# FelixWaiblinger/gym-pybullet-adrp

Measured on AMD Instinct MI355X. Metric: env-steps/sec (N parallel drones) at 1/2/4/8 MI355X; % HBM roofline, higher is better.
Workload: dtype f64; 1 GPU; HoverAviary Physics.PYB 240/30 Hz (8 sub-steps), 4096 envs x 1 drone per GPU, RPM actions, auto-reset; envs_per_gpu=4096, global_envs=4096, drones_per_env=1, parallelism=env-sharded dp1

## Files before the change

### gym_pybullet_adrp_amd/csrc/hover_kernel.h

```cpp
#pragma once

#include "adrp_device.h"
#include "dslpid_core.h"

namespace adrp {

enum HoverField {
    HF_POS = 0, HF_QUAT = 3, HF_VEL = 7, HF_OMEGA = 10, HF_LAST_RPM = 13, HF_ANGV = 17,
    HF_LINK_QUAT = 20, HF_NBASE = 24,
    HF_PID = 24, HF_NPID = 9
};
enum HoverInt { HI_STEP = 0, HI_EPISODE = 1, HI_RING_HEAD = 2, HI_N = 3 };

template <typename Real>
struct HoverConst {
    int S, trunc_steps, link_lag, physics;
    Real dt, mass, inv_mass, gravity;
    Real ixx, iyy, izz, inv_ixx, inv_iyy, inv_izz;
    Real kf, km, hover_rpm;
    Real px[4], py[4], pz[4];
    Real gnd_kf, prop_r4, gnd_clip;
    Real drag[3];
    Real dyn_arm;
    Real coll_hh, coll_r, coll_zoff;
// ... 20 lines not shown
    c.dyn_arm = Real(0.028072139213105935);
    c.coll_hh = Real(0.0125); c.coll_r = Real(0.06); c.coll_zoff = Real(0);
    c.ang_max = Real(188.49555921538757);
    c.target[0] = Real(0); c.target[1] = Real(0); c.target[2] = Real(1);
    c.pid_grav = Real(0.338492); c.pid_inv4kf = Real(791139240.5063292);
    c.ctrl_dt = Real(0.03333333333333333); c.ctrl_hz = Real(30);
    c.speed_limit = 0.25f;
    return c;
}

template <typename Real>
struct HoverReset {
    Real init_xyz[3], init_rpy[3], n_xyz[3], n_rpy[3], n_vel[3], n_om[3];
};

constexpr int kStepBlock = 64;
constexpr int kResetFields = 16;
#ifndef ADRP_PERSIST_SPLIT
#define ADRP_PERSIST_SPLIT 1
#endif
#ifndef ADRP_HOVER_ANGLE_HELPERS
#define ADRP_HOVER_ANGLE_HELPERS 1
#endif
template <typename Real>
constexpr bool angle_helpers() { return ADRP_HOVER_ANGLE_HELPERS != 0 && sizeof(Real) == 8; }
template <typename Real>
constexpr int help_waves() { return angle_helpers<Real>() ? 3 : 1; }

template <typename Real>
struct HoverArgs {
    const HoverConst<Real>* c;
    const HoverReset<Real>* r;
    Real* f;
    float* ring;
    int32_t* ist;
    const float* act;
    float* obs;
    float* rew;
    uint8_t* term;
    uint8_t* trunc;
    float* tobs;
    const uint8_t* mask;
    int32_t* contact_count;
    uint64_t seed;
    int64_t env_offset;
    int E, B, D, autoreset;
// ... 35 lines not shown
}
template <typename Real>
__device__ __forceinline__ V3<Real> row2_fm(Q4<Real> q) {
    const Real x2 = q.x + q.x, y2 = q.y + q.y, z2 = q.z + q.z;
    const Real xx = q.x * x2;
    const Real wx = q.w * x2, wy = q.w * y2;
    return {fmx(q.x, z2, -wy), fmx(q.y, z2, wx), Real(1) - fmx(q.y, y2, xx)};
}

template <typename Real>
struct Chain {
    V3<Real> wb;
    Real wn;
    V3<Real> zs;
    V3<Real> zc;
    V3<Real> m3;
    V3<Real> dti;
    M3<Real> R, Rs;
};

__device__ __forceinline__ float clamp100_(float x) { return __builtin_amdgcn_fmed3f(x, -100.0f, 100.0f); }
__device__ __forceinline__ double clamp100_(double x) { return clamp100_sel(x); }

template <typename Real>
__device__ __forceinline__ void clamp100_body(Q4<Real> q, V3<Real>& wb, Real& wn, V3<Real>& v, const ChainK<Real>& K) {
    const Real c = K.c100;
    const bool fast = wn > c;
    bool big = fast;
    if constexpr (sizeof(Real) == 8) {
        const bool bx = fabs_(v.x) > c, by = fabs_(v.y) > c, bz = fabs_(v.z) > c;
        big = fast | bx | by | bz;
    } else {
        v = v3(clamp100_(v.x), clamp100_(v.y), clamp100_(v.z));
    }
    if (__builtin_expect(__any(big), 0)) {
        if constexpr (sizeof(Real) == 8) v = v3(clamp100_(v.x), clamp100_(v.y), clamp100_(v.z));
        const M3<Real> R = rot_fm(q);
        const V3<Real> w = mul(R, wb);
        const V3<Real> wc = mulT(R, v3(clamp100_(w.x), clamp100_(w.y), clamp100_(w.z)));
        const Real wnc = hsqrt_nn_(dot(wc, wc), K);
        wb = v3(fast ? wc.x : wb.x, fast ? wc.y : wb.y, fast ? wc.z : wb.z);
        wn = fast ? wnc : wn;
    }
}

template <typename Real>
__device__ __forceinline__ bool flat_props(const HoverConst<Real>& a) {
    bool flat = true;
#pragma unroll
    for (int i = 0; i < 4; ++i) flat = flat && __builtin_constant_p(a.pz[i]) && a.pz[i] == Real(0);
    return flat;
}

template <typename Real, int PH, bool EXT = false>
__device__ __forceinline__ bool pyb_substep(const HoverConst<Real>& a, Body<Real>& b, Chain<Real>& st,
                                            const Real rpm[4], Real sum_f, V3<Real> P, Real tau_z,
                                            const ChainK<Real>& K, V3<Real> Fext = V3<Real>{}, Real* vxy = nullptr) {
    constexpr bool GND = (PH == ADRP_PHYS_PYB_GND || PH == ADRP_PHYS_PYB_GND_DRAG_DW);
    constexpr bool DRAG = (PH == ADRP_PHYS_PYB_DRAG || PH == ADRP_PHYS_PYB_GND_DRAG_DW);
    constexpr bool FULL = DRAG && !GND;
    const V3<Real> zs = st.zs;
    V3<Real> Fw = v3(sum_f * zs.x, sum_f * zs.y, sum_f * zs.z - a.mass * a.gravity);
    const V3<Real> m3 = st.m3;
    V3<Real> nb = flat_props(a)
                      ? v3(fmx(tau_z, m3.x, P.y * m3.z), fmx(tau_z, m3.y, -(P.x * m3.z)),
                           fmx(tau_z, m3.z, fmx(P.x, m3.y, -(P.y * m3.x))))
                      : v3(fmx(tau_z, m3.x, fmx(P.y, m3.z, -(P.z * m3.y))), fmx(tau_z, m3.y, fmx(P.z, m3.x, -(P.x * m3.z))),
                           fmx(tau_z, m3.z, fmx(P.x, m3.y, -(P.y * m3.x))));
    if constexpr (GND) {
        const Real sqx = b.q.x * b.q.x, sqy = b.q.y * b.q.y, sqz = b.q.z * b.q.z, squ = b.q.w * b.q.w;
        const Real sarg = Real(-2) * (b.q.x * b.q.z - b.q.w * b.q.y);
        const Real den = squ - sqx - sqy + sqz, num = Real(2) * (b.q.y * b.q.z + b.q.w * b.q.x);
        const bool gate = fabs_(sarg) < Real(0.99999) && (den > Real(0) || (den == Real(0) && num == Real(0)));
        if (gate) {
            Real sg = 0;
            V3<Real> G = v3(Real(0), Real(0), Real(0));
            const V3<Real> r2 = row2_fm(b.q);
#pragma unroll
            for (int i = 0; i < 4; ++i) {
                Real h = b.pos.z + r2.x * a.px[i] + r2.y * a.py[i] + r2.z * a.pz[i];
                h = h < a.gnd_clip ? a.gnd_clip : h;
                const Real k = a.prop_r4 * rcp_(h);
                const Real g = a.gnd_kf * rpm[i] * rpm[i] * k * k;
                sg += g;
                G = G + v3(g * a.px[i], g * a.py[i], g * a.pz[i]);
            }
            Fw = Fw + sg * st.zc;
            nb = nb + v3(G.y, -G.x, Real(0));
        }
    }
    if constexpr (DRAG) {
        Real s = 0;
#pragma unroll
        for (int i = 0; i < 4; ++i) s += b.prev_rpm[i];
        s = s * Real(0.10471975511965977);
        const V3<Real> dw = v3(-a.drag[0] * s * b.vel.x, -a.drag[1] * s * b.vel.y, -a.drag[2] * s * b.vel.z);
        if constexpr (GND) Fw = Fw + dw;
        else Fw = Fw + mul(st.Rs, mulT(st.R, dw));
    }
    if constexpr (EXT) Fw = Fw + Fext;
    V3<Real> wb = st.wb;
    const V3<Real> Iw = v3(a.ixx * wb.x, a.iyy * wb.y, a.izz * wb.z);
    const Real kw = K.k004 + K.k004 * st.wn;
    const V3<Real> rhs = v3(fmx(wb.z, Iw.y, fmx(-wb.y, Iw.z, fmx(-kw, Iw.x, nb.x))),
                            fmx(wb.x, Iw.z, fmx(-wb.z, Iw.x, fmx(-kw, Iw.y, nb.y))),
                            fmx(wb.y, Iw.x, fmx(-wb.x, Iw.y, fmx(-kw, Iw.z, nb.z))));
    const Real kv = K.k004 + K.k004 * hsqrt_nn_(dot(b.vel, b.vel), K);
    const V3<Real> acc = v3(fmx(-kv, b.vel.x, a.inv_mass * Fw.x), fmx(-kv, b.vel.y, a.inv_mass * Fw.y),
                            fmx(-kv, b.vel.z, a.inv_mass * Fw.z));
    wb = v3(fmx(st.dti.x, rhs.x, wb.x), fmx(st.dti.y, rhs.y, wb.y), fmx(st.dti.z, rhs.z, wb.z));
    b.vel = v3(b.vel.x + a.dt * acc.x, b.vel.y + a.dt * acc.y, b.vel.z + a.dt * acc.z);
    Real ang = hsqrt_nn_(dot(wb, wb), K);
    clamp100_body(b.q, wb, ang, b.vel, K);
    st.wb = wb;
    st.wn = ang;
    if (vxy) {
        vxy[0] = b.vel.x; vxy[1] = b.vel.y;
        b.pos.z = fmx(a.dt, b.vel.z, b.pos.z);
    } else {
        b.pos = v3(fmx(a.dt, b.vel.x, b.pos.x), fmx(a.dt, b.vel.y, b.pos.y), fmx(a.dt, b.vel.z, b.pos.z));
    }
    if (ang > a.ang_max) ang = a.ang_max;
    Real sinc, ch;
    expmap_sinc_cos(Real(0.5) * ang * a.dt, &sinc, &ch, K);
    const Real sc = (Real(0.5) * a.dt) * sinc;
    const V3<Real> ax = sc * wb;
    const Q4<Real> q0 = b.q;
    const Q4<Real> q1 = {ch * q0.x + ax.x * q0.w + ax.z * q0.y - ax.y * q0.z,
                         ch * q0.y + ax.y * q0.w + ax.x * q0.z - ax.z * q0.x,
                         ch * q0.z + ax.z * q0.w + ax.y * q0.x - ax.x * q0.y,
                         ch * q0.w - ax.x * q0.x - ax.y * q0.y - ax.z * q0.z};
    const Real inv = quat_inv_norm(q1.x * q1.x + q1.y * q1.y + q1.z * q1.z + q1.w * q1.w, K);
    if (a.link_lag) {
        b.ql = q0;
        st.zs = st.zc;
        const Real s2 = (inv + inv) * inv;
        st.m3 = v3(s2 * (ax.x * ax.z - ch * ax.y), s2 * (ax.y * ax.z + ch * ax.x),
                   Real(1) - s2 * (ax.x * ax.x + ax.y * ax.y));
        if constexpr (FULL) st.Rs = st.R;
    }
    b.q = {q1.x * inv, q1.y * inv, q1.z * inv, q1.w * inv};
    if constexpr (FULL) {
        st.R = rot_fm(b.q);
        st.zc = col2(st.R);
    } else {
        st.zc = col2_fm(b.q);
    }
    if (!a.link_lag) {
        st.zs = st.zc;
        st.m3 = v3(Real(0), Real(0), Real(1));
        if constexpr (FULL) st.Rs = st.R;
    }
    if (__builtin_expect(__any(b.pos.z + a.coll_zoff <= a.coll_hh + a.coll_r + Real(1e-6)), 0)) {
        const Real low = b.pos.z + a.coll_zoff - a.coll_hh * fabs_(st.zc.z) -
                         a.coll_r * hsqrt_nn_(st.zc.x * st.zc.x + st.zc.y * st.zc.y);
        if (low < Real(0)) {
            b.pos.z -= low;
            if (b.vel.z < Real(0)) b.vel.z = Real(0);
            return true;
        }
    }
    return false;
}

template <typename Real>
__device__ __forceinline__ void dyn_substep(const HoverConst<Real>& a, Body<Real>& b, const Real rpm[4]) {
    const M3<Real> R = rot(b.q);
    Real f[4], zt[4], sum = 0;
#pragma unroll
    for (int i = 0; i < 4; ++i) {
        f[i] = rpm[i] * rpm[i] * a.kf;
        zt[i] = rpm[i] * rpm[i] * a.km;
        sum += f[i];
    }
    const V3<Real> zb = col2(R);
    const V3<Real> force_w = v3(sum * zb.x, sum * zb.y, sum * zb.z - a.gravity * a.mass);
    const Real tz = -zt[0] + zt[1] - zt[2] + zt[3];
    const Real tx = (f[0] + f[1] - f[2] - f[3]) * a.dyn_arm;
    const Real ty = (-f[0] + f[1] + f[2] - f[3]) * a.dyn_arm;
    const V3<Real> rr = b.w;
    const V3<Real> tq = v3(tx, ty, tz) - cross(rr, v3(a.ixx * rr.x, a.iyy * rr.y, a.izz * rr.z));
    const V3<Real> rdd = v3(tq.x * a.inv_ixx, tq.y * a.inv_iyy, tq.z * a.inv_izz);
    b.vel = b.vel + a.dt * (a.inv_mass * force_w);
// ... 276 lines not shown
#pragma unroll
    for (int i = 0; i < n; ++i) {
        o[first + i] = off;
        if (i + 1 < n) off = field_lane(off + stride);
    }
}
template <typename Real>
struct BodyOffs {
    uint32_t o[HF_NBASE];
};
template <typename Real>
__device__ __forceinline__ BodyOffs<Real> body_offsets(int E, int e, bool lag, bool drag, bool dyn) {
    BodyOffs<Real> r;
    const uint32_t stride = uint32_t(E) * uint32_t(sizeof(Real)), off0 = uint32_t(e) * uint32_t(sizeof(Real));
    field_run(off0, stride, HF_POS, HF_LAST_RPM - HF_POS, r.o);
    if (drag) field_run(off0, stride, HF_LAST_RPM, 4, r.o);
    if (dyn) field_run(off0, stride, HF_ANGV, 3, r.o);
    if (lag) field_run(off0, stride, HF_LINK_QUAT, 4, r.o);
    return r;
}

template <typename Real>
__device__ __forceinline__ void load_body_at(const Real* f, const BodyOffs<Real>& k, Body<Real>& b, bool lag,
                                             bool drag, bool dyn) {
    b.pos = v3(field_at(f, k.o[HF_POS + 0]), field_at(f, k.o[HF_POS + 1]), field_at(f, k.o[HF_POS + 2]));
    b.q = {field_at(f, k.o[HF_QUAT + 0]), field_at(f, k.o[HF_QUAT + 1]), field_at(f, k.o[HF_QUAT + 2]),
           field_at(f, k.o[HF_QUAT + 3])};
    b.vel = v3(field_at(f, k.o[HF_VEL + 0]), field_at(f, k.o[HF_VEL + 1]), field_at(f, k.o[HF_VEL + 2]));
    b.w = v3(field_at(f, k.o[HF_OMEGA + 0]), field_at(f, k.o[HF_OMEGA + 1]), field_at(f, k.o[HF_OMEGA + 2]));
    if (lag) b.ql = {field_at(f, k.o[HF_LINK_QUAT + 0]), field_at(f, k.o[HF_LINK_QUAT + 1]),
                     field_at(f, k.o[HF_LINK_QUAT + 2]), field_at(f, k.o[HF_LINK_QUAT + 3])};
    else b.ql = b.q;
#pragma unroll
    for (int i = 0; i < 4; ++i) b.prev_rpm[i] = drag ? field_at(f, k.o[HF_LAST_RPM + i]) : Real(0);
    if (dyn) b.angv = v3(field_at(f, k.o[HF_ANGV + 0]), field_at(f, k.o[HF_ANGV + 1]), field_at(f, k.o[HF_ANGV + 2]));
    else b.angv = v3(Real(0), Real(0), Real(0));
}
template <typename Real>
__device__ __forceinline__ void store_body_at(Real* f, const BodyOffs<Real>& k, const Body<Real>& b, bool lag,
                                              bool drag, bool dyn) {
    field_last(f, k.o[HF_POS + 0]) = b.pos.x; field_last(f, k.o[HF_POS + 1]) = b.pos.y; field_last(f, k.o[HF_POS + 2]) = b.pos.z;
    field_last(f, k.o[HF_QUAT + 0]) = b.q.x; field_last(f, k.o[HF_QUAT + 1]) = b.q.y;
    field_last(f, k.o[HF_QUAT + 2]) = b.q.z; field_last(f, k.o[HF_QUAT + 3]) = b.q.w;
    field_last(f, k.o[HF_VEL + 0]) = b.vel.x; field_last(f, k.o[HF_VEL + 1]) = b.vel.y; field_last(f, k.o[HF_VEL + 2]) = b.vel.z;
    field_last(f, k.o[HF_OMEGA + 0]) = b.w.x; field_last(f, k.o[HF_OMEGA + 1]) = b.w.y; field_last(f, k.o[HF_OMEGA + 2]) = b.w.z;
    if (lag) {
        field_last(f, k.o[HF_LINK_QUAT + 0]) = b.ql.x; field_last(f, k.o[HF_LINK_QUAT + 1]) = b.ql.y;
        field_last(f, k.o[HF_LINK_QUAT + 2]) = b.ql.z; field_last(f, k.o[HF_LINK_QUAT + 3]) = b.ql.w;
    }
    if (drag) {
#pragma unroll
// ... 37 lines not shown
        store_body_at(f, body_offsets<Real>(E, e, lag, drag, dyn), b, lag, drag, dyn);
        field_form_end();
        return;
    }
    f[(HF_POS + 0) * E + e] = b.pos.x; f[(HF_POS + 1) * E + e] = b.pos.y; f[(HF_POS + 2) * E + e] = b.pos.z;
    f[(HF_QUAT + 0) * E + e] = b.q.x; f[(HF_QUAT + 1) * E + e] = b.q.y;
    f[(HF_QUAT + 2) * E + e] = b.q.z; f[(HF_QUAT + 3) * E + e] = b.q.w;
    f[(HF_VEL + 0) * E + e] = b.vel.x; f[(HF_VEL + 1) * E + e] = b.vel.y; f[(HF_VEL + 2) * E + e] = b.vel.z;
    f[(HF_OMEGA + 0) * E + e] = b.w.x; f[(HF_OMEGA + 1) * E + e] = b.w.y; f[(HF_OMEGA + 2) * E + e] = b.w.z;
    if (lag) {
        f[(HF_LINK_QUAT + 0) * E + e] = b.ql.x; f[(HF_LINK_QUAT + 1) * E + e] = b.ql.y;
        f[(HF_LINK_QUAT + 2) * E + e] = b.ql.z; f[(HF_LINK_QUAT + 3) * E + e] = b.ql.w;
    }
    if (drag) {
#pragma unroll
        for (int i = 0; i < 4; ++i) f[(HF_LAST_RPM + i) * E + e] = b.prev_rpm[i];
    }
    if (dyn) {
        f[(HF_ANGV + 0) * E + e] = b.angv.x; f[(HF_ANGV + 1) * E + e] = b.angv.y; f[(HF_ANGV + 2) * E + e] = b.angv.z;
    }
}

struct NoExtForce {};
template <typename Real, int PH, int SC, bool DRAG, typename Ext>
__device__ __forceinline__ bool pyb_chain(const HoverConst<Real>& C, Body<Real>& b, const Real rpm_in[4], bool lag,
                                          Ext ext, V3<Real>* wb_out = nullptr, Real* vxy = nullptr) {
    constexpr bool EXT = !__is_same(Ext, NoExtForce);
    const Real rpm[4] = {rpm_in[0], rpm_in[1], rpm_in[2], rpm_in[3]};
    Real sum_f = 0, t2 = 0;
    V3<Real> P = v3(Real(0), Real(0), Real(0));
#pragma unroll
    for (int i = 0; i < 4; ++i) {
        const Real r2 = rpm[i] * rpm[i];
        const Real f = r2 * C.kf;
        sum_f += f;
        const bool pz0 = __builtin_constant_p(C.pz[i]) && C.pz[i] == Real(0);
        const Real fx = f * C.px[i], fy = f * C.py[i], fz = f * C.pz[i];
        P = v3(P.x + fx, P.y + fy, pz0 ? P.z : P.z + fz);
        t2 += (i & 1) ? -r2 : r2;
    }
    const Real tau_z = t2 * C.km;
    ChainK<Real> K = chain_consts<Real>();
    HoverConst<Real> Cp = C;
    if constexpr (sizeof(Real) == 8) {
        pin_all(K);
        pin(Cp.dt); pin(Cp.mass); pin(Cp.gravity); pin(Cp.inv_mass); pin(Cp.ang_max);
        pin(Cp.ixx); pin(Cp.iyy); pin(Cp.izz); pin(Cp.inv_ixx); pin(Cp.inv_iyy); pin(Cp.inv_izz);
        pin(Cp.coll_hh); pin(Cp.coll_r); pin(Cp.coll_zoff);
    }
    Chain<Real> st{};
    {
        const M3<Real> R = rot_fm(b.q);
        const M3<Real> Rs = lag ? rot_fm(b.ql) : R;
        st.wb = mulT(R, b.w);
        st.zc = col2(R);
        st.zs = col2(Rs);
        st.m3 = lag ? mulT(R, st.zs) : v3(Real(0), Real(0), Real(1));
        if constexpr (DRAG) {
            st.R = R;
            st.Rs = Rs;
        }
    }
    st.wn = hsqrt_nn_(dot(b.w, b.w), K);
    st.dti = v3(Cp.dt * Cp.inv_ixx, Cp.dt * Cp.inv_iyy, Cp.dt * Cp.inv_izz);
    bool touched = false;
    auto substep = [&](int s) {
        if constexpr (EXT) touched |= pyb_substep<Real, PH, true>(Cp, b, st, rpm, sum_f, P, tau_z, K, ext(b, st));
        else touched |= pyb_substep<Real, PH>(Cp, b, st, rpm, sum_f, P, tau_z, K, V3<Real>{}, vxy ? vxy + 2 * s : nullptr);
#pragma unroll
        for (int i = 0; i < 4; ++i) b.prev_rpm[i] = rpm[i];
    };
    if constexpr (SC > 0) {
#pragma unroll
        for (int s = 0; s < SC; ++s) substep(s);
    } else {
        for (int s = 0; s < C.S; ++s) substep(s);
    }
    if (wb_out) *wb_out = st.wb;
    else b.w = mul(rot_fm(b.q), st.wb);
    return touched;
}

constexpr int kRowF4 = 18;

template <int A, int B>
__device__ __forceinline__ void stage_row(float4* lds_row, const float o12[12], const float (&ring)[B][A], int head1) {
    lds_row[0] = make_float4(o12[0], o12[1], o12[2], o12[3]);
    lds_row[1] = make_float4(o12[4], o12[5], o12[6], o12[7]);
    lds_row[2] = make_float4(o12[8], o12[9], o12[10], o12[11]);
#pragma unroll
// ... 12 lines not shown
    constexpr bool DRAG = (PH == ADRP_PHYS_PYB_DRAG || PH == ADRP_PHYS_PYB_GND_DRAG_DW);
    constexpr bool DYN = (PH == ADRP_PHYS_DYN);
    static_assert(!HELP || STG, "the reset helper wave pairs with the staged (all lanes live) kernel");
    constexpr bool ANG = HELP && angle_helpers<Real>();
    __shared__ Real rs_body[HELP ? kResetFields * kStepBlock : 1];
    __shared__ float rs_obs[HELP && !ANG ? 12 * kStepBlock : 1];
    constexpr int kResetObs = kStepBlock * kRowF4;
    __shared__ float4 rows[STG ? kStepBlock * kRowF4 + (ANG ? 3 * kStepBlock : 0) : 1];
    __shared__ Real ang_q[ANG ? 4 * kStepBlock : 1];
    __shared__ Real ang_r[ANG ? kStepBlock : 1];
    __shared__ Real ang_p[ANG ? kStepBlock : 1];
    __shared__ float ang_y[ANG ? kStepBlock : 1];
    constexpr int kWaves = HELP ? 1 + help_waves<Real>() : 1;
    constexpr auto cb = [](int w) { return w == 0 ? 0 : (w >= kWaves ? kRowF4 : (kWaves == 2 ? kRowF4 / 2 : 6 * (w - 1))); };
    constexpr bool TROWS = ANG;
    constexpr int kHelpLanes = 3 * kStepBlock, kRingF4 = kRowF4 - 3;
    constexpr int kRingPer = kStepBlock * kRingF4 / kHelpLanes;
    constexpr int kTermRows = kHelpLanes / kRowF4;
    static_assert(!TROWS || (kWaves == 4 && kRingPer * kHelpLanes == kStepBlock * kRingF4 && cb(1) == 0),
                  "copy-out over three helper waves");
    __shared__ int done_cnt[1];
    __shared__ uint8_t done_list[TROWS ? kStepBlock : 1];
    __shared__ uint8_t done_b[TROWS ? kStepBlock : 1];
    struct TailIdx {
        uint32_t ring[kRingPer], kin, fix, flag, sub, tcol;
    };
    [[maybe_unused]] auto tail_index = [&](int tl, int wv) {
        TailIdx t;
        const uint32_t g = uint32_t(wv - 1) * kStepBlock + uint32_t(tl);
#pragma unroll
        for (int j = 0; j < kRingPer; ++j) {
            const uint32_t n = g + kHelpLanes * uint32_t(j);
            const uint32_t row = (n * 4370u) >> 16;
            t.ring[j] = (row * kRowF4 + 3u + (n - kRingF4 * row)) * 16u;
            asm volatile("" : "+v"(t.ring[j]));
        }
        t.flag = (g * 21846u) >> 16;
        t.kin = (t.flag * kRowF4 + (g - 3u * t.flag)) * 16u;
        t.fix = (kResetObs + g) * 16u;
        t.sub = (g * 3641u) >> 16;
        t.tcol = g - kRowF4 * t.sub;
        asm volatile("" : "+v"(t.kin), "+v"(t.fix), "+v"(t.flag), "+v"(t.sub), "+v"(t.tcol));
        return t;
    };
    [[maybe_unused]] auto helper_ring = [&](const TailIdx& ti) {
        const char* lds = reinterpret_cast<const char*>(rows);
// ... 10 lines not shown
        const uint8_t fl = done_b[ti.flag];
        const char* lds = reinterpret_cast<const char*>(rows);
        char* dst = reinterpret_cast<char*>(a.obs) + size_t(blockIdx.x) * (kStepBlock * kRowF4 * sizeof(float4));
        const float4 o = *reinterpret_cast<const float4*>(lds + (fl ? ti.fix : ti.kin));
        float4 t0 = rows[row0 * kRowF4 + int(ti.tcol)];
        hold(t0.x); hold(t0.y); hold(t0.z); hold(t0.w);
        store_out(reinterpret_cast<float4*>(dst + ti.kin), o);
        const int cnt = __builtin_amdgcn_readfirstlane(cnt_v);
        const int sub = int(ti.sub), c = int(ti.tcol);
        const bool mine = sub < kTermRows;
        float4* tb = reinterpret_cast<float4*>(a.tobs) + size_t(blockIdx.x) * kStepBlock * kRowF4;
        if (mine && sub < cnt) tb[row0 * kRowF4 + c] = t0;
        for (int base = kTermRows; base < cnt && base < kStepBlock; base += kTermRows) {
            const int n = base + sub;
            if (mine && n < cnt) {
                const int row = done_list[n] & (kStepBlock - 1);
                tb[row * kRowF4 + c] = rows[row * kRowF4 + c];
            }
        }
    };
    if constexpr (HELP) {
        if (ANG && threadIdx.x >= 2 * kStepBlock) {
            const int tl = threadIdx.x & (kStepBlock - 1), wv = threadIdx.x / kStepBlock;
            AngK ak = ang_consts();
            pin_all(ak);
            const TailIdx ti = tail_index(tl, wv);
            __syncthreads();
            const Q4<Real> q = {ang_q[tl], ang_q[kStepBlock + tl], ang_q[2 * kStepBlock + tl], ang_q[3 * kStepBlock + tl]};
            if constexpr (ANG) {
                float* rowf = reinterpret_cast<float*>(rows) + tl * (4 * kRowF4);
                if (wv == 2) {
                    const double p = euler_pitch_lean(q, ak);
                    ang_p[tl] = p;
                    rowf[4] = float(p);
                } else {
                    const float y = float(euler_yaw_lean(q, ak));
                    ang_y[tl] = y;
                    rowf[5] = y;
                }
            }
            if constexpr (TROWS) helper_ring(ti);
            __syncthreads();
            __syncthreads();
            if constexpr (TROWS) {
                helper_tail(ti);
                return;
            }
            float4* dst = reinterpret_cast<float4*>(a.obs) + size_t(blockIdx.x) * kStepBlock * kRowF4;
            for (int k = cb(wv); k < cb(wv + 1); ++k) store_out(dst + tl + kStepBlock * k, rows[tl + kStepBlock * k]);
            return;
        }
        if (threadIdx.x >= kStepBlock) {
            const int tl = threadIdx.x - kStepBlock;
            const int he = blockIdx.x * kStepBlock + tl;
            const int E = a.E;
            const float4 av = reinterpret_cast<const float4*>(a.act)[he];
            float rg[BR][4];
#pragma unroll
            for (int p = 0; p < B; ++p) {
                const float4 v = reinterpret_cast<const float4*>(a.ring)[size_t(p) * E + he];
                rg[p][0] = v.x; rg[p][1] = v.y; rg[p][2] = v.z; rg[p][3] = v.w;
            }
            const int32_t head = a.ist[HI_RING_HEAD * E + he];
            int32_t hsc = 0, hep = a.ist[HI_EPISODE * E + he];
            Body<Real> rb;
            hover_reset_state(a, C, he, rb, hsc, hep);
            float o[12];
            hover_obs12(C, rb, o);
            const Real v[kResetFields] = {rb.pos.x, rb.pos.y, rb.pos.z, rb.q.x, rb.q.y, rb.q.z, rb.q.w,
                                          rb.vel.x, rb.vel.y, rb.vel.z, rb.w.x, rb.w.y, rb.w.z,
                                          rb.angv.x, rb.angv.y, rb.angv.z};
#pragma unroll
            for (int k = 0; k < kResetFields; ++k) rs_body[k * kStepBlock + tl] = v[k];
            if constexpr (ANG) {
                rows[kResetObs + 3 * tl + 0] = make_float4(o[0], o[1], o[2], o[3]);
                rows[kResetObs + 3 * tl + 1] = make_float4(o[4], o[5], o[6], o[7]);
                rows[kResetObs + 3 * tl + 2] = make_float4(o[8], o[9], o[10], o[11]);
            } else {
// ... 40 lines not shown
                helper_tail(ti);
                return;
            }
            float4* dst = reinterpret_cast<float4*>(a.obs) + size_t(blockIdx.x) * kStepBlock * kRowF4;
#pragma unroll
            for (int k = cb(1); k < cb(2); ++k) store_out(dst + tl + kStepBlock * k, rows[tl + kStepBlock * k]);
            return;
        }
    }
    const int E = a.E;
    const bool split = ADRP_PERSIST_SPLIT && !STG && !HELP && E == 1;
    const int e = split ? 0 : int(blockIdx.x) * kStepBlock + int(threadIdx.x);
    const int D = B > 0 ? 12 + B * A : a.D;
    if (e >= E) return;
    RACE_MARK(t0);
    const bool fit = FO == 2 ? field_offsets_fit<Real>(E) : FO == 1;
    const bool lag = C.link_lag && !DYN;
    const BodyOffs<Real> fo = body_offsets<Real>(E, e, lag, DRAG, DYN);
    uint32_t io[HI_N];
    field_run(uint32_t(e) * 4u, uint32_t(E) * 4u, 0, HI_N, io);
    Body<Real> b;
    int32_t sc, ep, head_ld;
    if (fit) {
        load_body_at<Real>(a.f, fo, b, lag, DRAG, DYN);
        sc = field_at(a.ist, io[HI_STEP]); ep = field_at(a.ist, io[HI_EPISODE]); head_ld = field_at(a.ist, io[HI_RING_HEAD]);
        field_form_end();
    } else {
        load_body(a, e, b, lag, DRAG, DYN);
        sc = a.ist[HI_STEP * E + e]; ep = a.ist[HI_EPISODE * E + e]; head_ld = a.ist[HI_RING_HEAD * E + e];
    }
    const int32_t head = head_ld;
    float act[A];
    if constexpr (SYS == 2) {
#pragma unroll
        for (int j = 0; j < A; ++j) act[j] = pre[j];
    } else if constexpr (SYS == 1) {
        uint32_t* sa = const_cast<uint32_t*>(reinterpret_cast<const uint32_t*>(a.act)) + size_t(e) * A;
#pragma unroll
        for (int j = 0; j < A; ++j)
            act[j] = __uint_as_float(__hip_atomic_load(sa + j, __ATOMIC_RELAXED, __HIP_MEMORY_SCOPE_SYSTEM));
    } else if constexpr (A == 4) {
        const float4 v = reinterpret_cast<const float4*>(a.act)[e];
        act[0] = v.x; act[1] = v.y; act[2] = v.z; act[3] = v.w;
    } else {
#pragma unroll
        for (int j = 0; j < A; ++j) act[j] = a.act[e * A + j];
    }
    float ring[BR][A];
#pragma unroll
    for (int p = 0; p < (HELP ? 0 : B); ++p) {
        if constexpr (A == 4) {
            const float4 v = reinterpret_cast<const float4*>(a.ring)[size_t(p) * E + e];
// ... 12 lines not shown
        if (fit) {
#pragma unroll
            for (int k = 0; k < HF_NPID; ++k) ctl[k] = field_at(a.f, po[HF_PID + k]);
            field_form_end();
        } else {
#pragma unroll
            for (int k = 0; k < HF_NPID; ++k) ctl[k] = a.f[(HF_PID + k) * E + e];
        }
        dslpid_rpm<Real, CTL>(C, b, act, ctl, rpm);
        if (fit) {
#pragma unroll
            for (int k = 0; k < HF_NPID; ++k) field_last(a.f, po[HF_PID + k]) = ctl[k];
            field_form_end();
        } else {
#pragma unroll
            for (int k = 0; k < HF_NPID; ++k) a.f[(HF_PID + k) * E + e] = ctl[k];
        }
    } else {
#pragma unroll
        for (int i = 0; i < 4; ++i) rpm[i] = C.hover_rpm * Real(rpm_gain(act[A == 1 ? 0 : i]));
    }
    bool touched = false;
    V3<Real> wbf = v3(Real(0), Real(0), Real(0));
    constexpr bool LATE_XY = ANG && !DYN && SC > 0;
    Real vxy[LATE_XY ? 2 * SC : 2] = {};
#ifdef ADRP_RACE_TIMING
    __builtin_amdgcn_s_waitcnt(0);
#endif
    RACE_MARK(t1);
    if constexpr (DYN) {
        if constexpr (SC > 0) {
#pragma unroll
            for (int s = 0; s < SC; ++s) dyn_substep(C, b, rpm);
        } else {
            for (int s = 0; s < C.S; ++s) dyn_substep(C, b, rpm);
        }
    } else {
        touched = pyb_chain<Real, PH, SC, DRAG>(C, b, rpm, lag, NoExtForce{}, ANG ? &wbf : nullptr, LATE_XY ? vxy : nullptr);
    }
    RACE_MARK(t2);
    if (touched && a.contact_count && (!split || threadIdx.x == 0)) atomicAdd(a.contact_count, 1);
    if constexpr (HELP) {
    } else if constexpr (A == 4)
        reinterpret_cast<float4*>(a.ring)[size_t(head) * E + e] = make_float4(act[0], act[1], act[2], act[3]);
    else
#pragma unroll
        for (int j = 0; j < A; ++j) a.ring[(size_t(head) * E + e) * A + j] = act[j];
    const int BB = B > 0 ? B : a.B;
    const int head1 = head + 1 == BB ? 0 : head + 1;
    auto store_state = [&]() {
        if (fit) {
            store_body_at<Real>(a.f, fo, b, lag, DRAG, DYN);
            field_last(a.ist, io[HI_STEP]) = sc;
            field_last(a.ist, io[HI_EPISODE]) = ep;
            field_last(a.ist, io[HI_RING_HEAD]) = head1;
            field_form_end();
        } else {
            store_body(a, e, b, lag, DRAG, DYN);
            a.ist[HI_STEP * E + e] = sc;
            a.ist[HI_EPISODE * E + e] = ep;
            a.ist[HI_RING_HEAD * E + e] = head1;
        }
    };
    float o12[12];
    V3<Real> rpy;
    if constexpr (ANG) {
        const int tl = threadIdx.x;
        ang_q[tl] = b.q.x; ang_q[kStepBlock + tl] = b.q.y; ang_q[2 * kStepBlock + tl] = b.q.z;
        ang_q[3 * kStepBlock + tl] = b.q.w;
        __syncthreads();
        hold(b.q.x); hold(b.q.y); hold(b.q.z); hold(b.q.w);
        hold(wbf.x); hold(wbf.y); hold(wbf.z);
        hold(b.pos.x); hold(b.pos.y); hold(b.pos.z);
        if constexpr (LATE_XY) {
#pragma unroll
            for (int k = 0; k < 2 * SC; ++k) hold(vxy[k]);
#pragma unroll
            for (int s = 0; s < SC; ++s) {
                b.pos.x = fmx(C.dt, vxy[2 * s], b.pos.x);
                b.pos.y = fmx(C.dt, vxy[2 * s + 1], b.pos.y);
            }
        }
        hold(b.vel.x); hold(b.vel.y); hold(b.vel.z);
        if constexpr (!DYN) b.w = mul(rot_fm(b.q), wbf);
        const V3<Real> w = C.physics == ADRP_PHYS_DYN ? b.angv : b.w;
        o12[0] = float(b.pos.x); o12[1] = float(b.pos.y); o12[2] = float(b.pos.z);
        o12[6] = float(b.vel.x); o12[7] = float(b.vel.y); o12[8] = float(b.vel.z);
        o12[9] = float(w.x);     o12[10] = float(w.y);    o12[11] = float(w.z);
    } else if (split) {
        rpy = hover_obs12_split(C, b, o12);
    } else {
        rpy = hover_obs12(C, b, o12);
    }
    const Real dx = C.target[0] - b.pos.x, dy = C.target[1] - b.pos.y, dz = C.target[2] - b.pos.z;
    const Real d2 = dx * dx + dy * dy + dz * dz;
    const Real r = Real(2) - d2 * d2;
    a.rew[e] = float(r > Real(0) ? r : Real(0));
    const bool te = d2 < Real(1e-8);
    bool tr = fabs_(b.pos.x) > Real(1.5) || fabs_(b.pos.y) > Real(1.5) || b.pos.z > Real(2.0) || sc >= C.trunc_steps;
    [[maybe_unused]] bool slow = false;
    if constexpr (ANG) {
        hold(b.w.x); hold(b.w.y); hold(b.w.z);
#pragma unroll
        for (int k = 0; k < 12; ++k)
            if (k < 3 || k > 5) hold(o12[k]);
        TruncK tk = trunc_consts();
        pin_all(tk);
        bool over = false;
        const bool sure = trunc_from_quat(b.q, tk, over);
        slow = __any(!sure);
        if (__builtin_expect(slow, 0)) {
            __syncthreads();
            rpy.x = ang_r[threadIdx.x];
            rpy.y = ang_p[threadIdx.x];
            over = fabs_(rpy.x) > Real(0.4) || fabs_(rpy.y) > Real(0.4);
        }
        tr = tr || over;
    } else {
        tr = tr || fabs_(rpy.x) > Real(0.4) || fabs_(rpy.y) > Real(0.4);
    }
    a.term[e] = te;
    a.trunc[e] = tr;
    sc += C.S;
    const bool done = a.autoreset && (te || tr);
    RACE_MARK(t3);
#ifdef ADRP_RACE_TIMING
    const unsigned long long dmask = __ballot(done);
    uint64_t t4 = 0;
#endif
    if constexpr (STG) {
        static_assert(A == 4 && B == 15, "staged rows: 72-float rows only");
        float4* my = rows + threadIdx.x * kRowF4;
        const int hu = __builtin_amdgcn_readfirstlane(head);
        if constexpr (HELP) {
        } else if (__all(head == hu)) {
            const int h1 = hu + 1 == B ? 0 : hu + 1;
#pragma unroll
            for (int p = 0; p < B; ++p) {
                const int k = p >= h1 ? p - h1 : p - h1 + B;
                my[3 + k] = make_float4(ring[p][0], ring[p][1], ring[p][2], ring[p][3]);
            }
            my[3 + B - 1] = make_float4(act[0], act[1], act[2], act[3]);
        } else {
#pragma unroll
            for (int p = 0; p < B; ++p) {
                const bool hit = p == head;
#pragma unroll
                for (int j = 0; j < A; ++j) ring[p][j] = hit ? act[j] : ring[p][j];
            }
            stage_row<A, B>(my, o12, ring, head1);
        }
        if constexpr (TROWS) {
            float* mf = reinterpret_cast<float*>(my);
            mf[0] = o12[0]; mf[1] = o12[1]; mf[2] = o12[2];
            mf[6] = o12[6]; mf[7] = o12[7];
            my[2] = make_float4(o12[8], o12[9], o12[10], o12[11]);
            const unsigned long long done_mask = __ballot(done);
            done_b[threadIdx.x] = done;
            done_cnt[0] = a.tobs ? __popcll(done_mask) : 0;
            if (done) {
                const uint32_t rank = __builtin_amdgcn_mbcnt_hi(uint32_t(done_mask >> 32), __builtin_amdgcn_mbcnt_lo(uint32_t(done_mask), 0u));
                done_list[rank] = uint8_t(threadIdx.x);
                const int t = threadIdx.x;
                Real v[kResetFields];
#pragma unroll
                for (int k = 0; k < kResetFields; ++k) v[k] = rs_body[k * kStepBlock + t];
                b.pos = v3(v[0], v[1], v[2]);
                b.q = {v[3], v[4], v[5], v[6]};
                b.ql = b.q;
                b.vel = v3(v[7], v[8], v[9]);
                b.w = v3(v[10], v[11], v[12]);
                b.angv = v3(v[13], v[14], v[15]);
#pragma unroll
                for (int i = 0; i < 4; ++i) b.prev_rpm[i] = Real(0);
                sc = 0;
                ep += 1;
            }
            RACE_SET(t4);
            store_state();
// ... 137 lines not shown
```

Before: 790.0 million env-steps/s.

## Split translational integration onto a helper wave fed via LDS slots

Moves the translational half of each PyBullet sub-step (velocity/position update, drag, velocity clamp, ground contact, reward and bounds flags) onto a dedicated helper wavefront. The main wave now integrates only rotation and hands the body z-axis for each sub-step to the helper through shared-memory slots with per-slot ready flags and spin-waits. The goal is to shorten the serial dependency chain and the register load on the main wave by overlapping the two halves. In exchange it adds extra shared memory, spin-wait synchronisation and barriers, and a more fragile schedule between waves.

```diff
diff --git a/gym_pybullet_adrp_amd/csrc/hover_kernel.h b/gym_pybullet_adrp_amd/csrc/hover_kernel.h
--- a/gym_pybullet_adrp_amd/csrc/hover_kernel.h
+++ b/gym_pybullet_adrp_amd/csrc/hover_kernel.h
@@ -66,6 +66,9 @@
 #ifndef ADRP_HOVER_ANGLE_HELPERS
 #define ADRP_HOVER_ANGLE_HELPERS 1
 #endif
+#ifndef ADRP_HOVER_TRANS_WAVE
+#define ADRP_HOVER_TRANS_WAVE 1
+#endif
 template <typename Real>
 constexpr bool angle_helpers() { return ADRP_HOVER_ANGLE_HELPERS != 0 && sizeof(Real) == 8; }
 template <typename Real>
@@ -147,19 +150,20 @@
 __device__ __forceinline__ float clamp100_(float x) { return __builtin_amdgcn_fmed3f(x, -100.0f, 100.0f); }
 __device__ __forceinline__ double clamp100_(double x) { return clamp100_sel(x); }
 
-template <typename Real>
+template <typename Real, bool VEL = true>
 __device__ __forceinline__ void clamp100_body(Q4<Real> q, V3<Real>& wb, Real& wn, V3<Real>& v, const ChainK<Real>& K) {
     const Real c = K.c100;
     const bool fast = wn > c;
     bool big = fast;
-    if constexpr (sizeof(Real) == 8) {
+    if constexpr (!VEL) {
+    } else if constexpr (sizeof(Real) == 8) {
         const bool bx = fabs_(v.x) > c, by = fabs_(v.y) > c, bz = fabs_(v.z) > c;
         big = fast | bx | by | bz;
     } else {
         v = v3(clamp100_(v.x), clamp100_(v.y), clamp100_(v.z));
     }
     if (__builtin_expect(__any(big), 0)) {
-        if constexpr (sizeof(Real) == 8) v = v3(clamp100_(v.x), clamp100_(v.y), clamp100_(v.z));
+        if constexpr (VEL && sizeof(Real) == 8) v = v3(clamp100_(v.x), clamp100_(v.y), clamp100_(v.z));
         const M3<Real> R = rot_fm(q);
         const V3<Real> w = mul(R, wb);
         const V3<Real> wc = mulT(R, v3(clamp100_(w.x), clamp100_(w.y), clamp100_(w.z)));
@@ -168,6 +172,16 @@
         wn = fast ? wnc : wn;
     }
 }
+template <typename Real>
+__device__ __forceinline__ void clamp100_vel(V3<Real>& v, const ChainK<Real>& K) {
+    if constexpr (sizeof(Real) == 8) {
+        const Real c = K.c100;
+        const bool bx = fabs_(v.x) > c, by = fabs_(v.y) > c, bz = fabs_(v.z) > c;
+        if (__builtin_expect(__any(bx | by | bz), 0)) v = v3(clamp100_(v.x), clamp100_(v.y), clamp100_(v.z));
+    } else {
+        v = v3(clamp100_(v.x), clamp100_(v.y), clamp100_(v.z));
+    }
+}
 
 template <typename Real>
 __device__ __forceinline__ bool flat_props(const HoverConst<Real>& a) {
@@ -177,13 +191,14 @@
     return flat;
 }
 
-template <typename Real, int PH, bool EXT = false>
+template <typename Real, int PH, bool EXT = false, bool ROT = false>
 __device__ __forceinline__ bool pyb_substep(const HoverConst<Real>& a, Body<Real>& b, Chain<Real>& st,
                                             const Real rpm[4], Real sum_f, V3<Real> P, Real tau_z,
                                             const ChainK<Real>& K, V3<Real> Fext = V3<Real>{}, Real* vxy = nullptr) {
     constexpr bool GND = (PH == ADRP_PHYS_PYB_GND || PH == ADRP_PHYS_PYB_GND_DRAG_DW);
     constexpr bool DRAG = (PH == ADRP_PHYS_PYB_DRAG || PH == ADRP_PHYS_PYB_GND_DRAG_DW);
     constexpr bool FULL = DRAG && !GND;
+    static_assert(!ROT || (!GND && !DRAG && !EXT), "the rotational half stands alone in plain PYB only");
     const V3<Real> zs = st.zs;
     V3<Real> Fw = v3(sum_f * zs.x, sum_f * zs.y, sum_f * zs.z - a.mass * a.gravity);
     const V3<Real> m3 = st.m3;
@@ -230,16 +245,20 @@
     const V3<Real> rhs = v3(fmx(wb.z, Iw.y, fmx(-wb.y, Iw.z, fmx(-kw, Iw.x, nb.x))),
                             fmx(wb.x, Iw.z, fmx(-wb.z, Iw.x, fmx(-kw, Iw.y, nb.y))),
                             fmx(wb.y, Iw.x, fmx(-wb.x, Iw.y, fmx(-kw, Iw.z, nb.z))));
-    const Real kv = K.k004 + K.k004 * hsqrt_nn_(dot(b.vel, b.vel), K);
-    const V3<Real> acc = v3(fmx(-kv, b.vel.x, a.inv_mass * Fw.x), fmx(-kv, b.vel.y, a.inv_mass * Fw.y),
-                            fmx(-kv, b.vel.z, a.inv_mass * Fw.z));
+    V3<Real> acc{};
+    if constexpr (!ROT) {
+        const Real kv = K.k004 + K.k004 * hsqrt_nn_(dot(b.vel, b.vel), K);
+        acc = v3(fmx(-kv, b.vel.x, a.inv_mass * Fw.x), fmx(-kv, b.vel.y, a.inv_mass * Fw.y),
+                 fmx(-kv, b.vel.z, a.inv_mass * Fw.z));
+    }
     wb = v3(fmx(st.dti.x, rhs.x, wb.x), fmx(st.dti.y, rhs.y, wb.y), fmx(st.dti.z, rhs.z, wb.z));
-    b.vel = v3(b.vel.x + a.dt * acc.x, b.vel.y + a.dt * acc.y, b.vel.z + a.dt * acc.z);
+    if constexpr (!ROT) b.vel = v3(b.vel.x + a.dt * acc.x, b.vel.y + a.dt * acc.y, b.vel.z + a.dt * acc.z);
     Real ang = hsqrt_nn_(dot(wb, wb), K);
-    clamp100_body(b.q, wb, ang, b.vel, K);
+    clamp100_body<Real, !ROT>(b.q, wb, ang, b.vel, K);
     st.wb = wb;
     st.wn = ang;
-    if (vxy) {
+    if constexpr (ROT) {
+    } else if (vxy) {
         vxy[0] = b.vel.x; vxy[1] = b.vel.y;
         b.pos.z = fmx(a.dt, b.vel.z, b.pos.z);
     } else {
@@ -276,6 +295,7 @@
         st.m3 = v3(Real(0), Real(0), Real(1));
         if constexpr (FULL) st.Rs = st.R;
     }
+    if constexpr (ROT) return false;
     if (__builtin_expect(__any(b.pos.z + a.coll_zoff <= a.coll_hh + a.coll_r + Real(1e-6)), 0)) {
         const Real low = b.pos.z + a.coll_zoff - a.coll_hh * fabs_(st.zc.z) -
                          a.coll_r * hsqrt_nn_(st.zc.x * st.zc.x + st.zc.y * st.zc.y);
@@ -284,6 +304,33 @@
             if (b.vel.z < Real(0)) b.vel.z = Real(0);
             return true;
         }
+    }
+    return false;
+}
+
+template <typename Real>
+__device__ __forceinline__ void pyb_trans_substep(const HoverConst<Real>& a, V3<Real>& pos, V3<Real>& vel, V3<Real> zs,
+                                                  Real sum_f, const ChainK<Real>& K) {
+    const V3<Real> Fw = v3(sum_f * zs.x, sum_f * zs.y, sum_f * zs.z - a.mass * a.gravity);
+    const Real kv = K.k004 + K.k004 * hsqrt_nn_(dot(vel, vel), K);
+    const V3<Real> acc = v3(fmx(-kv, vel.x, a.inv_mass * Fw.x), fmx(-kv, vel.y, a.inv_mass * Fw.y),
+                            fmx(-kv, vel.z, a.inv_mass * Fw.z));
+    vel = v3(vel.x + a.dt * acc.x, vel.y + a.dt * acc.y, vel.z + a.dt * acc.z);
+    clamp100_vel(vel, K);
+    pos = v3(fmx(a.dt, vel.x, pos.x), fmx(a.dt, vel.y, pos.y), fmx(a.dt, vel.z, pos.z));
+}
+template <typename Real>
+__device__ __forceinline__ bool pyb_trans_near_plane(const HoverConst<Real>& a, V3<Real> pos) {
+    return __builtin_expect(__any(pos.z + a.coll_zoff <= a.coll_hh + a.coll_r + Real(1e-6)), 0);
+}
+template <typename Real>
+__device__ __forceinline__ bool pyb_trans_contact(const HoverConst<Real>& a, V3<Real>& pos, V3<Real>& vel, V3<Real> zc) {
+    const Real low = pos.z + a.coll_zoff - a.coll_hh * fabs_(zc.z) -
+                     a.coll_r * hsqrt_nn_(zc.x * zc.x + zc.y * zc.y);
+    if (low < Real(0)) {
+        pos.z -= low;
+        if (vel.z < Real(0)) vel.z = Real(0);
+        return true;
     }
     return false;
 }
@@ -606,11 +653,13 @@
 
 template <typename Real>
 __device__ __forceinline__ void load_body_at(const Real* f, const BodyOffs<Real>& k, Body<Real>& b, bool lag,
-                                             bool drag, bool dyn) {
-    b.pos = v3(field_at(f, k.o[HF_POS + 0]), field_at(f, k.o[HF_POS + 1]), field_at(f, k.o[HF_POS + 2]));
+                                             bool drag, bool dyn, bool kin = true) {
+    if (kin) b.pos = v3(field_at(f, k.o[HF_POS + 0]), field_at(f, k.o[HF_POS + 1]), field_at(f, k.o[HF_POS + 2]));
+    else b.pos = v3(Real(0), Real(0), Real(0));
     b.q = {field_at(f, k.o[HF_QUAT + 0]), field_at(f, k.o[HF_QUAT + 1]), field_at(f, k.o[HF_QUAT + 2]),
            field_at(f, k.o[HF_QUAT + 3])};
-    b.vel = v3(field_at(f, k.o[HF_VEL + 0]), field_at(f, k.o[HF_VEL + 1]), field_at(f, k.o[HF_VEL + 2]));
+    if (kin) b.vel = v3(field_at(f, k.o[HF_VEL + 0]), field_at(f, k.o[HF_VEL + 1]), field_at(f, k.o[HF_VEL + 2]));
+    else b.vel = v3(Real(0), Real(0), Real(0));
     b.w = v3(field_at(f, k.o[HF_OMEGA + 0]), field_at(f, k.o[HF_OMEGA + 1]), field_at(f, k.o[HF_OMEGA + 2]));
     if (lag) b.ql = {field_at(f, k.o[HF_LINK_QUAT + 0]), field_at(f, k.o[HF_LINK_QUAT + 1]),
                      field_at(f, k.o[HF_LINK_QUAT + 2]), field_at(f, k.o[HF_LINK_QUAT + 3])};
@@ -694,10 +743,13 @@
 }
 
 struct NoExtForce {};
-template <typename Real, int PH, int SC, bool DRAG, typename Ext>
+struct NoHandOff {};
+template <typename Real, int PH, int SC, bool DRAG, typename Ext, typename Hand = NoHandOff>
 __device__ __forceinline__ bool pyb_chain(const HoverConst<Real>& C, Body<Real>& b, const Real rpm_in[4], bool lag,
-                                          Ext ext, V3<Real>* wb_out = nullptr, Real* vxy = nullptr) {
+                                          Ext ext, V3<Real>* wb_out = nullptr, Real* vxy = nullptr, Hand hand = Hand{}) {
     constexpr bool EXT = !__is_same(Ext, NoExtForce);
+    constexpr bool HAND = !__is_same(Hand, NoHandOff);
+    static_assert(!HAND || (!EXT && !DRAG && SC > 0 && PH == ADRP_PHYS_PYB), "the hand-off is plain PYB's");
     const Real rpm[4] = {rpm_in[0], rpm_in[1], rpm_in[2], rpm_in[3]};
     Real sum_f = 0, t2 = 0;
     V3<Real> P = v3(Real(0), Real(0), Real(0));
@@ -735,9 +787,16 @@
     }
     st.wn = hsqrt_nn_(dot(b.w, b.w), K);
     st.dti = v3(Cp.dt * Cp.inv_ixx, Cp.dt * Cp.inv_iyy, Cp.dt * Cp.inv_izz);
+    if constexpr (HAND) {
+        hand(0, st.zs);
+        hand(1, st.zc);
+    }
     bool touched = false;
     auto substep = [&](int s) {
-        if constexpr (EXT) touched |= pyb_substep<Real, PH, true>(Cp, b, st, rpm, sum_f, P, tau_z, K, ext(b, st));
+        if constexpr (HAND) {
+            pyb_substep<Real, PH, false, true>(Cp, b, st, rpm, sum_f, P, tau_z, K);
+            hand(s + 2, st.zc);
+        } else if constexpr (EXT) touched |= pyb_substep<Real, PH, true>(Cp, b, st, rpm, sum_f, P, tau_z, K, ext(b, st));
         else touched |= pyb_substep<Real, PH>(Cp, b, st, rpm, sum_f, P, tau_z, K, V3<Real>{}, vxy ? vxy + 2 * s : nullptr);
 #pragma unroll
         for (int i = 0; i < 4; ++i) b.prev_rpm[i] = rpm[i];
@@ -796,6 +855,38 @@
     __shared__ int done_cnt[1];
     __shared__ uint8_t done_list[TROWS ? kStepBlock : 1];
     __shared__ uint8_t done_b[TROWS ? kStepBlock : 1];
+    constexpr bool TW = TROWS && PH == ADRP_PHYS_PYB && CTL == 0 && SC > 0 && ADRP_HOVER_TRANS_WAVE != 0;
+    constexpr int kSlots = SC + 2, kTwOut = HF_VEL + 3;
+    using Real2 = Real __attribute__((ext_vector_type(2)));
+    __shared__ Real2 tw_zxy[TW ? kSlots * kStepBlock : 1];
+    __shared__ Real tw_zz[TW ? kSlots * kStepBlock : 1];
+    __shared__ int tw_mark[TW ? kSlots : 1];
+    __shared__ Real tw_out[TW ? kTwOut * kStepBlock : 1];
+    __shared__ uint8_t tw_flag[TW ? kStepBlock : 1];
+#ifdef ADRP_RACE_TIMING
+    __shared__ unsigned long long tw_time[1];
+#endif
+    [[maybe_unused]] auto slot_wait = [&](int k) {
+        while (__builtin_amdgcn_readfirstlane(__hip_atomic_load(&tw_mark[k], __ATOMIC_RELAXED, __HIP_MEMORY_SCOPE_WORKGROUP)) == 0)
+            __builtin_amdgcn_s_sleep(1);
+        asm volatile("" ::: "memory");
+    };
+    [[maybe_unused]] auto slot_read = [&](int k, int tl) {
+        const Real2 xy = tw_zxy[k * kStepBlock + tl];
+        return v3(Real(xy.x), Real(xy.y), tw_zz[k * kStepBlock + tl]);
+    };
+    [[maybe_unused]] auto slot_write = [&](int k, V3<Real> z) {
+        const int tl = threadIdx.x;
+        if (k == 0) __builtin_amdgcn_s_barrier();
+        Real2 xy;
+        xy.x = z.x; xy.y = z.y;
+        tw_zxy[k * kStepBlock + tl] = xy;
+        tw_zz[k * kStepBlock + tl] = z.z;
+        if (k > 0) {
+            asm volatile("" ::: "memory");
+            __hip_atomic_store(&tw_mark[k], 1, __ATOMIC_RELAXED, __HIP_MEMORY_SCOPE_WORKGROUP);
+        }
+    };
     struct TailIdx {
         uint32_t ring[kRingPer], kin, fix, flag, sub, tcol;
     };
@@ -852,13 +943,89 @@
     if constexpr (HELP) {
         if (ANG && threadIdx.x >= 2 * kStepBlock) {
             const int tl = threadIdx.x & (kStepBlock - 1), wv = threadIdx.x / kStepBlock;
+            [[maybe_unused]] const bool trans = TW && __builtin_amdgcn_readfirstlane(wv) == 3;
+            [[maybe_unused]] V3<Real> tp{}, tv{};
+            [[maybe_unused]] float4 tact = make_float4(0.0f, 0.0f, 0.0f, 0.0f);
+            [[maybe_unused]] float trew = 0.0f;
+            [[maybe_unused]] bool tterm = false;
+            if constexpr (TW) {
+                if (trans) {
+                    const int te_ = int(blockIdx.x) * kStepBlock + tl;
+                    auto fld = [&](int k) {
+                        if constexpr (FO == 1) return field_at(a.f, (uint32_t(k) * uint32_t(a.E) + uint32_t(te_)) * uint32_t(sizeof(Real)));
+                        else return a.f[size_t(k) * a.E + te_];
+                    };
+                    tp = v3(fld(HF_POS + 0), fld(HF_POS + 1), fld(HF_POS + 2));
+                    tv = v3(fld(HF_VEL + 0), fld(HF_VEL + 1), fld(HF_VEL + 2));
+                    tact = reinterpret_cast<const float4*>(a.act)[te_];
+                    if (tl < kSlots) __hip_atomic_store(&tw_mark[tl], 0, __ATOMIC_RELAXED, __HIP_MEMORY_SCOPE_WORKGROUP);
+                    asm volatile("" ::: "memory");
+                    __builtin_amdgcn_s_waitcnt(0xc07f);
+                }
+                __builtin_amdgcn_s_barrier();
+            }
             AngK ak = ang_consts();
             pin_all(ak);
             const TailIdx ti = tail_index(tl, wv);
+            if constexpr (TW) {
+                if (trans) {
+                    const bool lag = C.link_lag;
+                    ChainK<Real> K = chain_consts<Real>();
+                    HoverConst<Real> Cp = C;
+                    pin(K.k004); pin(K.c100); pin(K.nn_min);
+                    pin(Cp.dt); pin(Cp.mass); pin(Cp.gravity); pin(Cp.inv_mass);
+                    pin(Cp.coll_hh); pin(Cp.coll_r); pin(Cp.coll_zoff);
+                    const float ta[4] = {tact.x, tact.y, tact.z, tact.w};
+                    Real sum_f = 0;
+#pragma unroll
+                    for (int i = 0; i < 4; ++i) {
+                        const Real rpm = C.hover_rpm * Real(rpm_gain(ta[i]));
+                        const Real r2 = rpm * rpm;
+                        const Real f = r2 * C.kf;
+                        sum_f += f;
+                    }
+                    bool touched = false;
+#pragma unroll
+                    for (int s = 0; s < SC; ++s) {
+                        const int k = lag ? s : s + 1;
+                        slot_wait(k > 0 ? k : 1);
+                        pyb_trans_substep(Cp, tp, tv, slot_read(k, tl), sum_f, K);
+                        if (pyb_trans_near_plane(Cp, tp)) {
+                            slot_wait(s + 2);
+                            touched |= pyb_trans_contact(Cp, tp, tv, slot_read(s + 2, tl));
+                        }
+                    }
+                    if (touched && a.contact_count) atomicAdd(a.contact_count, 1);
+                    const Real dx = C.target[0] - tp.x, dy = C.target[1] - tp.y, dz = C.target[2] - tp.z;
+                    const Real d2 = dx * dx + dy * dy + dz * dz;
+                    const Real r = Real(2) - d2 * d2;
+                    trew = float(r > Real(0) ? r : Real(0));
+                    tterm = d2 < Real(1e-8);
+                    const bool te = tterm;
+                    const bool trp = fabs_(tp.x) > Real(1.5) || fabs_(tp.y) > Real(1.5) || tp.z > Real(2.0);
+                    tw_out[(HF_POS + 0) * kStepBlock + tl] = tp.x; tw_out[(HF_POS + 1) * kStepBlock + tl] = tp.y;
+                    tw_out[(HF_POS + 2) * kStepBlock + tl] = tp.z;
+                    tw_out[(HF_VEL + 0) * kStepBlock + tl] = tv.x; tw_out[(HF_VEL + 1) * kStepBlock + tl] = tv.y;
+                    tw_out[(HF_VEL + 2) * kStepBlock + tl] = tv.z;
+                    tw_flag[tl] = uint8_t((te ? 1 : 0) | (trp ? 2 : 0));
+#ifdef ADRP_RACE_TIMING
+                    if (tl == 0) tw_time[0] = __builtin_amdgcn_s_memtime();
+#endif
+                }
+            }
             __syncthreads();
             const Q4<Real> q = {ang_q[tl], ang_q[kStepBlock + tl], ang_q[2 * kStepBlock + tl], ang_q[3 * kStepBlock + tl]};
             if constexpr (ANG) {
                 float* rowf = reinterpret_cast<float*>(rows) + tl * (4 * kRowF4);
+                if constexpr (TW) {
+                    if (trans) {
+                        const int te_ = int(blockIdx.x) * kStepBlock + tl;
+                        a.rew[te_] = trew;
+                        a.term[te_] = tterm;
+                        rowf[0] = float(tp.x); rowf[1] = float(tp.y); rowf[2] = float(tp.z);
+                        rowf[6] = float(tv.x); rowf[7] = float(tv.y); rowf[8] = float(tv.z);
+                    }
+                }
                 if (wv == 2) {
                     const double p = euler_pitch_lean(q, ak);
                     ang_p[tl] = p;
@@ -884,6 +1051,7 @@
             const int tl = threadIdx.x - kStepBlock;
             const int he = blockIdx.x * kStepBlock + tl;
             const int E = a.E;
+            if constexpr (TW) __builtin_amdgcn_s_barrier();
             const float4 av = reinterpret_cast<const float4*>(a.act)[he];
             float rg[BR][4];
 #pragma unroll
@@ -970,12 +1138,13 @@
     Body<Real> b;
     int32_t sc, ep, head_ld;
     if (fit) {
-        load_body_at<Real>(a.f, fo, b, lag, DRAG, DYN);
+        load_body_at<Real>(a.f, fo, b, lag, DRAG, DYN, !TW);
         sc = field_at(a.ist, io[HI_STEP]); ep = field_at(a.ist, io[HI_EPISODE]); head_ld = field_at(a.ist, io[HI_RING_HEAD]);
         field_form_end();
     } else {
         load_body(a, e, b, lag, DRAG, DYN);
         sc = a.ist[HI_STEP * E + e]; ep = a.ist[HI_EPISODE * E + e]; head_ld = a.ist[HI_RING_HEAD * E + e];
+        if constexpr (TW) b.pos = b.vel = v3(Real(0), Real(0), Real(0));
     }
     const int32_t head = head_ld;
     float act[A];
@@ -1034,7 +1203,7 @@
     }
     bool touched = false;
     V3<Real> wbf = v3(Real(0), Real(0), Real(0));
-    constexpr bool LATE_XY = ANG && !DYN && SC > 0;
+    constexpr bool LATE_XY = ANG && !DYN && SC > 0 && !TW;
     Real vxy[LATE_XY ? 2 * SC : 2] = {};
 #ifdef ADRP_RACE_TIMING
     __builtin_amdgcn_s_waitcnt(0);
@@ -1047,6 +1216,8 @@
         } else {
             for (int s = 0; s < C.S; ++s) dyn_substep(C, b, rpm);
         }
+    } else if constexpr (TW) {
+        pyb_chain<Real, PH, SC, DRAG>(C, b, rpm, lag, NoExtForce{}, &wbf, nullptr, slot_write);
     } else {
         touched = pyb_chain<Real, PH, SC, DRAG>(C, b, rpm, lag, NoExtForce{}, ANG ? &wbf : nullptr, LATE_XY ? vxy : nullptr);
     }
@@ -1080,10 +1251,26 @@
         const int tl = threadIdx.x;
         ang_q[tl] = b.q.x; ang_q[kStepBlock + tl] = b.q.y; ang_q[2 * kStepBlock + tl] = b.q.z;
         ang_q[3 * kStepBlock + tl] = b.q.w;
+#ifdef ADRP_RACE_TIMING
+        [[maybe_unused]] const uint64_t t_a = __builtin_amdgcn_s_memtime();
+#endif
         __syncthreads();
+#ifdef ADRP_RACE_TIMING
+        if constexpr (TW) {
+            if (threadIdx.x == 0) {
+                const uint64_t t_w = tw_time[0];
+                atomicAdd(&g_race_phase[t_a >= t_w ? 20 : 21], (unsigned long long)(t_a >= t_w ? t_a - t_w : t_w - t_a));
+            }
+        }
+#endif
+        if constexpr (TW) {
+            const Real* src = tw_out + threadIdx.x;
+            b.pos = v3(src[(HF_POS + 0) * kStepBlock], src[(HF_POS + 1) * kStepBlock], src[(HF_POS + 2) * kStepBlock]);
+            b.vel = v3(src[(HF_VEL + 0) * kStepBlock], src[(HF_VEL + 1) * kStepBlock], src[(HF_VEL + 2) * kStepBlock]);
+        }
         hold(b.q.x); hold(b.q.y); hold(b.q.z); hold(b.q.w);
         hold(wbf.x); hold(wbf.y); hold(wbf.z);
-        hold(b.pos.x); hold(b.pos.y); hold(b.pos.z);
+        if constexpr (!TW) { hold(b.pos.x); hold(b.pos.y); hold(b.pos.z); }
         if constexpr (LATE_XY) {
 #pragma unroll
             for (int k = 0; k < 2 * SC; ++k) hold(vxy[k]);
@@ -1093,29 +1280,38 @@
                 b.pos.y = fmx(C.dt, vxy[2 * s + 1], b.pos.y);
             }
         }
-        hold(b.vel.x); hold(b.vel.y); hold(b.vel.z);
+        if constexpr (!TW) { hold(b.vel.x); hold(b.vel.y); hold(b.vel.z); }
         if constexpr (!DYN) b.w = mul(rot_fm(b.q), wbf);
         const V3<Real> w = C.physics == ADRP_PHYS_DYN ? b.angv : b.w;
-        o12[0] = float(b.pos.x); o12[1] = float(b.pos.y); o12[2] = float(b.pos.z);
-        o12[6] = float(b.vel.x); o12[7] = float(b.vel.y); o12[8] = float(b.vel.z);
+        if constexpr (!TW) {
+            o12[0] = float(b.pos.x); o12[1] = float(b.pos.y); o12[2] = float(b.pos.z);
+            o12[6] = float(b.vel.x); o12[7] = float(b.vel.y); o12[8] = float(b.vel.z);
+        }
         o12[9] = float(w.x);     o12[10] = float(w.y);    o12[11] = float(w.z);
     } else if (split) {
         rpy = hover_obs12_split(C, b, o12);
     } else {
         rpy = hover_obs12(C, b, o12);
     }
-    const Real dx = C.target[0] - b.pos.x, dy = C.target[1] - b.pos.y, dz = C.target[2] - b.pos.z;
-    const Real d2 = dx * dx + dy * dy + dz * dz;
-    const Real r = Real(2) - d2 * d2;
-    a.rew[e] = float(r > Real(0) ? r : Real(0));
-    const bool te = d2 < Real(1e-8);
-    bool tr = fabs_(b.pos.x) > Real(1.5) || fabs_(b.pos.y) > Real(1.5) || b.pos.z > Real(2.0) || sc >= C.trunc_steps;
+    bool te, tr;
+    if constexpr (TW) {
+        const uint8_t fl = tw_flag[threadIdx.x];
+        te = (fl & 1) != 0;
+        tr = (fl & 2) != 0 || sc >= C.trunc_steps;
+    } else {
+        const Real dx = C.target[0] - b.pos.x, dy = C.target[1] - b.pos.y, dz = C.target[2] - b.pos.z;
+        const Real d2 = dx * dx + dy * dy + dz * dz;
+        const Real r = Real(2) - d2 * d2;
+        a.rew[e] = float(r > Real(0) ? r : Real(0));
+        te = d2 < Real(1e-8);
+        tr = fabs_(b.pos.x) > Real(1.5) || fabs_(b.pos.y) > Real(1.5) || b.pos.z > Real(2.0) || sc >= C.trunc_steps;
+    }
     [[maybe_unused]] bool slow = false;
     if constexpr (ANG) {
         hold(b.w.x); hold(b.w.y); hold(b.w.z);
 #pragma unroll
         for (int k = 0; k < 12; ++k)
-            if (k < 3 || k > 5) hold(o12[k]);
+            if (TW ? k > 8 : (k < 3 || k > 5)) hold(o12[k]);
         TruncK tk = trunc_consts();
         pin_all(tk);
         bool over = false;
@@ -1131,7 +1327,7 @@
     } else {
         tr = tr || fabs_(rpy.x) > Real(0.4) || fabs_(rpy.y) > Real(0.4);
     }
-    a.term[e] = te;
+    if constexpr (!TW) a.term[e] = te;
     a.trunc[e] = tr;
     sc += C.S;
     const bool done = a.autoreset && (te || tr);
@@ -1164,9 +1360,13 @@
         }
         if constexpr (TROWS) {
             float* mf = reinterpret_cast<float*>(my);
-            mf[0] = o12[0]; mf[1] = o12[1]; mf[2] = o12[2];
-            mf[6] = o12[6]; mf[7] = o12[7];
-            my[2] = make_float4(o12[8], o12[9], o12[10], o12[11]);
+            if constexpr (TW) {
+                mf[9] = o12[9]; mf[10] = o12[10]; mf[11] = o12[11];
+            } else {
+                mf[0] = o12[0]; mf[1] = o12[1]; mf[2] = o12[2];
+                mf[6] = o12[6]; mf[7] = o12[7];
+                my[2] = make_float4(o12[8], o12[9], o12[10], o12[11]);
+            }
             const unsigned long long done_mask = __ballot(done);
             done_b[threadIdx.x] = done;
             done_cnt[0] = a.tobs ? __popcll(done_mask) : 0;
```

New measurement: 880.5 million env-steps/s, median of 6. 1.11x the previous value.
